# epfl-lts2/pygsp

Measured on AMD Instinct MI355X. Metric: filtered-vertices/sec (N·Nsig·K/s) + achieved HBM GB/s vs roofline, 1M-vertex K=30, higher is better.
Workload: dtype f64

## Files before the change

pygsp_amd/csrc/gspx_ctx.hip.h:

```cpp
#pragma once

struct Options {
  int64_t kernel = 0;
  int64_t vec = 0;
  int64_t rows_per_wave = 0;
  int64_t narrow_g_log2 = -1;
  int64_t waves_per_block = 4;
  int64_t calib_mix = 0;
  int64_t graph_launch = 2;
  int64_t tile_gather = 1;
  int64_t tile_workgroups = 0;
  int64_t knn_f32 = 1;
  int64_t tile_pad = 1;
  int64_t tile_min_row = 16;
  int64_t staged_copy = 1;
  int64_t staged_copy_min_mb = 32;
  int64_t copy_threads = 0;
  int64_t tile_regroup = 1;
  int64_t tile_acc_builds = 1;
  int64_t tile_lg = 0;
  int64_t edge_vertex_walk = 1;
  int64_t fuse_input = 1;
  int64_t tile_nt = -1;
  int64_t synthesis = 0;
  int64_t alternate_sweep = 1;
  int64_t xcd_remap = 1;
  int64_t combine = 0;
  int64_t ws_limit_mb = 65536;
  int64_t max_batch = 0;
  int64_t gather_rccl = 1;
  int64_t lds_pad_kb = 0;
  int64_t host_pipeline = 1;
  int64_t host_batch = 0;
  int64_t host_edge = 0;
  int64_t host_threads = 0;
  int64_t streamed_alloc = 1;
  int64_t layout_splits = 0;
};

struct gspx_ctx {
  int device = 0;
  int cu_count = 256;
  hipStream_t stream = nullptr;
  Options opt;
  DevMem ws_t;
  DevMem ws_r;
  DevMem ws_w;
  DevMem io_x, io_y;
  DevMem ws_spec;
  DevMem ws_sq, ws_sqp;
  HostPipe* pipe = nullptr;
  CopyStage* copy = nullptr;
  bool counted = false;
  std::mutex comms_mu;
  std::vector<struct gspx_comm*> comms;
  hipEvent_t ev[4] = {nullptr, nullptr, nullptr, nullptr};
  std::vector<hipEvent_t> ev_pool;
  double timing[5] = {0, 0, 0, 0, 0};
  int64_t step_kinds[2] = {0, 0};
  bool capturing = false;
  std::vector<unsigned char> seen_key;
  std::vector<unsigned char> graph_key;
  hipGraphExec_t graph_exec = nullptr;
  int64_t graph_kinds[2] = {0, 0};
};

static std::atomic<int> g_live_ctx[64];

static void replay_reset(gspx_ctx* ctx) {
  if (!ctx) return;
  ctx->seen_key.clear();
  ctx->graph_key.clear();
// ... 153 lines not shown
  ctx->ws_r.release();
  ctx->ws_w.release();
  ctx->io_x.release();
  ctx->io_y.release();
  ctx->ws_spec.release();
  ctx->ws_sq.release();
  ctx->ws_sqp.release();
  if (ctx->pipe) {
    ctx->pipe->destroy();
    delete ctx->pipe;
    ctx->pipe = nullptr;
  }
  if (ctx->copy) {
    ctx->copy->destroy();
    delete ctx->copy;
    ctx->copy = nullptr;
  }
  if (ctx->stream) (void)hipStreamDestroy(ctx->stream);
  delete ctx;
  return GSPX_OK;
}

extern "C" int gspx_ctx_sync(gspx_ctx* ctx) {
  if (!ctx) return set_err(GSPX_ERR_INVALID, "null ctx");
  HIPCHK(hipSetDevice(ctx->device));
  HIPCHK(hipStreamSynchronize(ctx->stream));
  return GSPX_OK;
}

struct OptionDef {
  const char* key;
  int64_t Options::*slot;
  bool (*ok)(int64_t);
  const char* refusal;
};
static const OptionDef OPTION_TABLE[] = {
    {"kernel", &Options::kernel, [](int64_t v) { return v == 0 || v == 1 || v == 2 || v == 5; },
     "kernel must be 0 (auto), 1 (panel), 2 (narrow) or 5 (LDS-staged)"},
    {"vec", &Options::vec, [](int64_t v) { return v == 0 || v == 1 || v == 2 || v == 4; }, "vec must be 0, 1, 2 or 4"},
    {"rows_per_wave", &Options::rows_per_wave, [](int64_t v) { return v >= 0 && v <= 1024; },
     "rows_per_wave must be in [0, 1024] (0 = auto)"},
    {"narrow_g_log2", &Options::narrow_g_log2, [](int64_t v) { return v >= -1 && v <= 6; },
     "narrow_g_log2 must be in [-1, 6] (-1 = auto)"},
    {"waves_per_block", &Options::waves_per_block, [](int64_t v) { return v == 4 || v == 8 || v == 16; },
     "waves_per_block must be 4, 8 or 16"},
    {"alternate_sweep", &Options::alternate_sweep, nullptr, nullptr},
    {"synthesis", &Options::synthesis, nullptr, nullptr},
    {"tile_gather", &Options::tile_gather, nullptr, nullptr},
    {"graph_launch", &Options::graph_launch, nullptr, nullptr},
    {"tile_workgroups", &Options::tile_workgroups, nullptr, nullptr},
    {"tile_lg", &Options::tile_lg, nullptr, nullptr},
    {"tile_regroup", &Options::tile_regroup, nullptr, nullptr},
    {"tile_acc_builds", &Options::tile_acc_builds, nullptr, nullptr},
    {"staged_copy", &Options::staged_copy, nullptr, nullptr},
    {"staged_copy_min_mb", &Options::staged_copy_min_mb, nullptr, nullptr},
    {"copy_threads", &Options::copy_threads, nullptr, nullptr},
    {"tile_min_row", &Options::tile_min_row, nullptr, nullptr},
    {"tile_pad", &Options::tile_pad, nullptr, nullptr},
    {"knn_f32", &Options::knn_f32, nullptr, nullptr},
    {"tile_nt", &Options::tile_nt, nullptr, nullptr},
    {"fuse_input", &Options::fuse_input, nullptr, nullptr},
    {"edge_vertex_walk", &Options::edge_vertex_walk, nullptr, nullptr},
    {"xcd_remap", &Options::xcd_remap, nullptr, nullptr},
    {"combine", &Options::combine, nullptr, nullptr},
    {"ws_limit_mb", &Options::ws_limit_mb, nullptr, nullptr},
    {"max_batch", &Options::max_batch, nullptr, nullptr},
    {"gather_rccl", &Options::gather_rccl, nullptr, nullptr},
    {"lds_pad_kb", &Options::lds_pad_kb, nullptr, nullptr},
    {"host_pipeline", &Options::host_pipeline, nullptr, nullptr},
    {"host_batch", &Options::host_batch, nullptr, nullptr},
    {"host_edge", &Options::host_edge, nullptr, nullptr},
    {"host_threads", &Options::host_threads, nullptr, nullptr},
    {"streamed_alloc", &Options::streamed_alloc, nullptr, nullptr},
    {"layout_splits", &Options::layout_splits, [](int64_t v) { return v >= 0 && v <= 65535; },
     "layout_splits must be in [0, 65535] (0 = automatic)"},
};

static const OptionDef* find_option(const char* key) {
  if (key)
    for (const OptionDef& d : OPTION_TABLE)
      if (!strcmp(key, d.key)) return &d;
  set_err(GSPX_ERR_INVALID, "unknown option '%s'", key ? key : "(null)");
  return nullptr;
}

extern "C" int gspx_ctx_set_option(gspx_ctx* ctx, const char* key, int64_t value) {
  replay_reset(ctx);
  if (!ctx) return set_err(GSPX_ERR_INVALID, "null ctx");
  const OptionDef* d = find_option(key);
  if (!d) return GSPX_ERR_INVALID;
  if (d->ok && !d->ok(value)) return set_err(GSPX_ERR_INVALID, "%s", d->refusal);
  ctx->opt.*d->slot = value;
  if (d->slot == &Options::streamed_alloc) {
    const bool on = value != 0;
    (void)hipSetDevice(ctx->device);
    for (DevMem* m : {&ctx->ws_t, &ctx->ws_r}) {
      if (!on && m->va_size) {
        (void)hipStreamSynchronize(ctx->stream);
        m->release();
      }
      m->streamed = on;
    }
  }
  return GSPX_OK;
}

// ... 200 lines not shown
```

pygsp_amd/csrc/gspx_poly.hip.h:

```cpp
#pragma once

struct PlanStep {
  double scale = 1.0, gamma = -1.0;
  int flush = 0;
  int final = 0;
  std::vector<double> w;
};

static void make_plan_fused(int nf, int M, const std::vector<double>& cp, bool acc_existing,
                            bool final_to_y, std::vector<PlanStep>& plan) {
  const int K = M - 1;
  plan.assign((size_t)K, PlanStep());
  int covered = -1;
  bool first = !acc_existing;
  for (int k = 1; k <= K; ++k) {
    PlanStep& st = plan[(size_t)k - 1];
    st.scale = (k == 1) ? 0.5 : 1.0;
    st.gamma = (k == 1) ? 0.0 : -1.0;
    st.w.assign((size_t)nf * 3, 0.0);
    const bool must = (k == K) || (k >= 2 && (k - 2) > covered);
    if (!must) continue;
    st.flush = first ? 1 : 2;
    first = false;
    st.final = (k == K && final_to_y) ? 1 : 0;
// ... 343 lines not shown
  return (int)std::max<int64_t>(1, std::min(std::min(tiles, want), fit));
}
static size_t cross_parts(const gspx_ctx* ctx, int N, unsigned w, int M, int nf) {
  size_t most = 0;
  for (int here : {std::min(nf, CROSS_PASS), nf % CROSS_PASS})
    for (int vec = 1; here > 0 && vec <= (w % 2 == 0 ? 2 : 1); ++vec)
      most = std::max(most, (size_t)cross_gx(ctx, N, w, M, here, vec) * (size_t)here * M * w);
  return most;
}

template <typename T>
static int launch_slot_cross_dots(gspx_ctx* ctx, const T* slots, int M, size_t slot_stride, unsigned pitch, int N,
                                  unsigned w, const int* perm, const CrossDots& cd, hipStream_t st) {
  const T* z = (const T*)cd.z;
  const int vec = cross_vec<T>(w, pitch, z, cd.ldz);
  const int cwl = sqnorm_cwl(w / vec);
  typedef void (*kern_t)(const T*, int, size_t, u32, const T*, int, size_t, u32, const int*, int, int, int, double*);
  for (int f0 = 0; f0 < cd.nf; f0 += CROSS_PASS) {
    const int here = std::min(CROSS_PASS, cd.nf - f0);
    const bool few = here <= CROSS_FEW;
    kern_t kern = few ? k_slot_cross_dots<T, 1, 16, CROSS_FEW> : k_slot_cross_dots<T, 1, 8, CROSS_PASS>;
    if constexpr (sizeof(T) == 4) {
      if (vec == 2) kern = few ? k_slot_cross_dots<T, 2, 8, CROSS_FEW> : k_slot_cross_dots<T, 2, 4, CROSS_PASS>;
    }
    const int gx = cross_gx(ctx, N, w, M, here, vec);
    const dim3 grid((unsigned)gx, (unsigned)cross_chunks(M, here, vec), (w / vec + (1u << cwl) - 1) >> cwl);
    hipLaunchKernelGGL(kern, grid, dim3(256), 0, st, slots, M, slot_stride, (u32)pitch, z + (size_t)f0 * cd.zplane, here,
                       cd.zplane, (u32)cd.ldz, perm, N, (int)w, cwl, cd.part);
    const int64_t n = (int64_t)here * M * w;
    hipLaunchKernelGGL(k_dots_reduce, dim3((unsigned)((n + 63) / 64)), dim3(256), 0, st, cd.part, gx, n, (int)w,
                       cd.out + (size_t)f0 * M * cd.ldo, cd.ldo);
  }
  return GSPX_OK;
}

struct SlotsUse {
  int (*fn)(gspx_ctx*, const void*, int, size_t, unsigned, int, unsigned, const int*, const void*, hipStream_t);
  const void* arg;
};

template <typename T> static bool tile_geometry(const gspx_graph* g, const Options& opt, unsigned ld) {
  constexpr int TVEC = 16 / (int)sizeof(T);
  const size_t U = (size_t)g->N * ld;
  return opt.tile_gather && g->gt_rows == GSPX_TILE_BR && (size_t)ld * sizeof(T) >= (size_t)opt.tile_min_row &&
         (ld % TVEC) == 0 && U * sizeof(T) < ((size_t)1 << 31) && (size_t)g->nnz_int * sizeof(T) < ((size_t)1 << 31);
}
template <typename T>
static bool tile_usable(const gspx_graph* g, const Options& opt, unsigned ld, const T* y, unsigned ldy) {
  constexpr int TVEC = 16 / (int)sizeof(T);
  return tile_geometry<T>(g, opt, ld) && (ldy % TVEC) == 0 && (((uintptr_t)y / sizeof(T)) % TVEC) == 0;
}
template <typename T>
static int launch_step_tile(gspx_graph* g, const Options& opt, TileArgs<T> t, unsigned ld, hipStream_t st,
                            const T* vals = nullptr) {
  const size_t rowb = (size_t)ld * sizeof(T);
  int lg = rowb <= 16 ? 1 : rowb <= 32 ? 2 : rowb <= 64 ? 4 : rowb <= 128 ? 8 : 16;
  if (opt.tile_lg == 8 || opt.tile_lg == 4 || opt.tile_lg == 2) lg = rowb <= 128 ? std::max(lg, (int)opt.tile_lg) : 16;
  const bool narrow = lg < 16;
  const int ncol = narrow ? 1 : (int)((rowb + 255) / 256);
  const int flavour = t.old_rows ? 1 : t.nin > 0 ? 2 : 0;
  typedef void (*kern_t)(const TileArgs<T>);
  static const kern_t wide[3][3] = {
      {k_step_tile<T, 0>, k_step_tile<T, 1>, k_step_tile<T, 2>},
      {k_step_tile<T, 0, 16, true>, k_step_tile<T, 1, 16, true>, k_step_tile<T, 2, 16, true>},
      {k_step_tile<T, 0, 16, false, true>, k_step_tile<T, 1, 16, false, true>, k_step_tile<T, 2, 16, false, true>}};
  static const kern_t slim[3][4] = {
      {k_step_tile<T, 1, 1, false, false, 64>, k_step_tile<T, 1, 2, false, false, 128>,
       k_step_tile<T, 1, 4, false, false, 256>, k_step_tile<T, 1, 8>},
      {k_step_tile<T, 1, 1, true, false, 64>, k_step_tile<T, 1, 2, true, false, 128>,
       k_step_tile<T, 1, 4, true, false, 256>, k_step_tile<T, 1, 8, true>},
      {k_step_tile<T, 1, 1, false, true, 64>, k_step_tile<T, 1, 2, false, true, 128>,
       k_step_tile<T, 1, 4, false, true, 256>, k_step_tile<T, 1, 8, false, true>}};
  kern_t kern = narrow ? slim[flavour][lg == 1 ? 0 : lg == 2 ? 1 : lg == 4 ? 2 : 3] : wide[flavour][ncol <= 2 ? ncol : 0];
  unsigned threads = narrow ? 64u * (unsigned)lg : 512u;
  const bool noacc = opt.tile_acc_builds && t.flush == 0 && !narrow && flavour == 0;
  if (noacc) {
    static const kern_t freek[3] = {k_step_tile<T, 0, 16, false, false, 512, 16, 0, false>,
                                    k_step_tile<T, 1, 16, false, false, 512, 16, 0, false>,
                                    k_step_tile<T, 2, 16, false, false, 512, 16, 0, false>};
    kern = freek[ncol <= 2 ? ncol : 0];
  }
  bool mix = false;
  if (opt.calib_mix && !narrow && flavour == 0) {
    static const kern_t mixk[2][3] = {
        {k_step_tile<T, 0, 16, false, false, 512, 16, 1>, k_step_tile<T, 1, 16, false, false, 512, 16, 1>,
         k_step_tile<T, 2, 16, false, false, 512, 16, 1>},
        {k_step_tile<T, 0, 16, false, false, 512, 16, 2>, k_step_tile<T, 1, 16, false, false, 512, 16, 2>,
         k_step_tile<T, 2, 16, false, false, 512, 16, 2>}};
    static const kern_t mixfree[2][3] = {
        {k_step_tile<T, 0, 16, false, false, 512, 16, 1, false>, k_step_tile<T, 1, 16, false, false, 512, 16, 1, false>,
         k_step_tile<T, 2, 16, false, false, 512, 16, 1, false>},
        {k_step_tile<T, 0, 16, false, false, 512, 16, 2, false>, k_step_tile<T, 1, 16, false, false, 512, 16, 2, false>,
         k_step_tile<T, 2, 16, false, false, 512, 16, 2, false>}};
    kern = (noacc ? mixfree : mixk)[opt.calib_mix == 2 ? 1 : 0][ncol <= 2 ? ncol : 0];
    mix = true;
  }
  const int pieces = (int)(rowb / 16);
  if (opt.tile_regroup && ncol == 1 && flavour != 1 && pieces < lg && !mix) {
#define GSPX_CL(LG_, CL_, NT_) \
  (flavour == 2 ? (kern_t)k_step_tile<T, 1, LG_, false, true, NT_, CL_> : (kern_t)k_step_tile<T, 1, LG_, false, false, NT_, CL_>)
    kern_t k2 = nullptr;
    unsigned nt2 = 0;
    if (lg == 4 && pieces == 3) k2 = GSPX_CL(4, 3, 192), nt2 = 192;
    else if (lg == 8 && pieces == 5) k2 = GSPX_CL(8, 5, 320), nt2 = 320;
    else if (lg == 16 && pieces == 10) k2 = GSPX_CL(16, 10, 320), nt2 = 320;
#undef GSPX_CL
    if (k2) kern = k2, threads = nt2;
  }
  size_t lds = g->gt_lds;
  if (lg < 8)
    lds = std::min(lds, (size_t)GSPX_TILE_MAXN1 * 16 * lg + (((size_t)g->gt_entmax * sizeof(T) + 15) & ~(size_t)15) +
                            (((size_t)g->gt_entmax + 15) & ~(size_t)15) + 64);
  if (lg < 8) lds = (lds + 2047) & ~(size_t)2047;
  int per_cu = 2;
  {
    struct Known { size_t attr = 0; std::map<size_t, int> fit; };
    static std::map<std::pair<const void*, int>, Known> known;
    static std::mutex lds_mu;
    std::lock_guard<std::mutex> lock(lds_mu);
    Known& k = known[std::make_pair((const void*)kern, g->ctx->device)];
    if (k.attr < lds) {
      HIPCHK(hipFuncSetAttribute((const void*)kern, hipFuncAttributeMaxDynamicSharedMemorySize, (int)lds));
      k.attr = lds;
    }
    if (lg < 8) {
      auto it = k.fit.find(lds);
      if (it == k.fit.end()) {
        int fit = 2;
        HIPCHK(hipOccupancyMaxActiveBlocksPerMultiprocessor(&fit, (const void*)kern, (int)threads, lds));
        it = k.fit.emplace(lds, std::max(2, std::min(fit, 16))).first;
      }
      per_cu = it->second;
    }
  }
// ... 93 lines not shown
  *width = max_ld;
  return GSPX_OK;
}

template <typename Batch>
static int run_batches(gspx_graph* g, int64_t Nsig, int64_t width, int steps, const Batch& batch) {
  gspx_ctx* ctx = g->ctx;
  size_t ev_idx = 0;
  HIPCHK(hipEventRecord(ctx->ev[0], ctx->stream));
  for (int64_t c0 = 0; c0 < Nsig; c0 += width)
    CHK(batch(c0, (unsigned)std::min<int64_t>(width, Nsig - c0), ev_idx));
  HIPCHK(hipEventRecord(ctx->ev[1], ctx->stream));
  HIPCHK(hipStreamSynchronize(ctx->stream));
  float ms = 0;
  HIPCHK(hipEventElapsedTime(&ms, ctx->ev[0], ctx->ev[1]));
  ctx->timing[0] = ms;
  double phase[3] = {0, 0, 0};
  for (size_t i = 0; i + 3 < ev_idx; i += 4)
    for (size_t j = 0; j < 3; ++j) {
      float t = 0;
      HIPCHK(hipEventElapsedTime(&t, ctx->ev_pool[i + j], ctx->ev_pool[i + j + 1]));
      phase[j] += t;
    }
  ctx->timing[1] = phase[1];
  ctx->timing[2] = (double)(ev_idx / 4) * steps;
  ctx->timing[3] = phase[0];
  ctx->timing[4] = phase[2];
  return GSPX_OK;
}

template <typename T>
static int run_batch(gspx_graph* g, int nf, int M, const std::vector<double>& cp, const T* x,
                     unsigned ldx, T* y, unsigned ldy, unsigned ld, bool deferred,
                     bool acc_existing, bool final_to_y, size_t& ev_idx, const SqNorms* sq = nullptr,
                     const SlotDots* sd = nullptr, const CrossDots* cd = nullptr, const SlotsUse* use = nullptr) {
  gspx_ctx* ctx = g->ctx;
  const Options& opt = ctx->opt;
  hipStream_t st = ctx->stream;
  const int N = (int)g->N;
  const int K = M - 1;
  const WorkPanels wp = work_panels<T>(g, opt, deferred || nf == 1, 1, ld, y, ldy);
  const bool tile_direct = wp.tile_direct, padded = wp.padded;
  const unsigned ldw = wp.ldw;
  const size_t U = (size_t)N * ldw;
  const Shape shape = choose_shape(opt, sizeof(T), ld, vec_cap(4, ldy, y));
  const int* perm = g->has_perm ? g->perm.as<int>() : nullptr;

  std::vector<PlanStep> plan;
  if (deferred)
    make_plan_deferred(nf, M, plan);
  else
    make_plan_fused(nf, M, cp, acc_existing, final_to_y, plan);

  std::vector<T> hw;
  if (deferred) {
    hw.resize((size_t)nf * M);
    for (size_t i = 0; i < hw.size(); ++i) hw[i] = (T)cp[i];
  } else {
    hw.resize((size_t)K * nf * 3);
    for (int k = 0; k < K; ++k)
      for (int j = 0; j < nf * 3; ++j) hw[(size_t)k * nf * 3 + j] = (T)plan[(size_t)k].w[(size_t)j];
  }
  const bool cap = ctx->capturing;
  if (!cap) {
    CHK(ctx->ws_w.ensure(hw.size() * sizeof(T) + 64));
    HIPCHK(hipMemcpyAsync(ctx->ws_w.p, hw.data(), hw.size() * sizeof(T), hipMemcpyHostToDevice, st));
    HIPCHK(hipStreamSynchronize(st));
  }

  const size_t nslots = deferred ? (size_t)M : 2;
  const size_t SU = U;
  CHK(ctx->ws_t.ensure(nslots * SU * sizeof(T) + 256));
  if (!deferred) CHK(ctx->ws_r.ensure((size_t)nf * U * sizeof(T) + 256));
  T* slots = ctx->ws_t.as<T>();
  T* racc = ctx->ws_r.as<T>();

  hipEvent_t ev[4] = {};
  if (!cap) CHK(batch_events(ctx, ev_idx, ev));
  const bool tile_ok = tile_direct || padded;
  const unsigned char* xb = (const unsigned char*)x;
  const unsigned char* yb = (const unsigned char*)y;
  const size_t xbytes = (size_t)N * ldx * sizeof(T), ybytes = (size_t)nf * N * ldy * sizeof(T);
  const bool fuse_in = tile_direct && !deferred && opt.fuse_input && g->gt_slow == 0 && ldx == ld &&
                       ((uintptr_t)x % 16) == 0 && (xb + xbytes <= yb || yb + ybytes <= xb) &&
                       (!g->has_perm || (g->gt_ns1 > 0 && (!cap || g->gt_s1nat.p)));
  if (fuse_in) {
    CHK(ensure_s1nat(g, st));
  } else if (padded) {
    const unsigned nb = (unsigned)std::min<size_t>((U + 255) / 256, 65536);
    hipLaunchKernelGGL((k_permute_in_pad<T>), dim3(nb), dim3(256), 0, st, x, ldx, slots, ldw, ld, N, perm);
  } else {
    launch_permute_in<T>(x, ldx, slots, ld, N, perm, vec_cap(shape.vec, ldx, x), st);
  }
  if (!cap) HIPCHK(hipEventRecord(ev[1], st));

  CHK(prepare_coff<T>(g, shape, ld, st));
  StepArgs<T> a = step_base<T>(g, ld, y, ldy);
  a.nf = nf;
  a.racc = racc;
  for (int k = 1; k <= K; ++k) {
    const PlanStep& ps = plan[(size_t)k - 1];
    if (tile_ok) {
      TileArgs<T> t{};
      if (deferred) {
        t.cur = slots + (size_t)(k - 1) * SU;
        t.old = (k >= 2 && ps.gamma != 0.0) ? slots + (size_t)(k - 2) * SU : t.cur;
        t.out = slots + (size_t)k * SU;
      } else {
        t.cur = slots + (size_t)((k - 1) & 1) * SU;
        t.old = ps.gamma == 0.0 ? t.cur : slots + (size_t)(k & 1) * SU;
        t.out = slots + (size_t)(k & 1) * SU;
        if (fuse_in && k == 1) {
          t.cur = x;
          t.old = x;
          t.s1rows = g->has_perm ? g->gt_s1nat.as<int>() : nullptr;
        } else if (fuse_in && k == 2) {
          t.old = x;
          t.old_rows = perm;
        }
      }
      t.racc = racc;
      t.y = y;
      t.ldy = ldy;
      t.perm = perm;
      t.scale = (T)ps.scale;
      t.gamma = (T)ps.gamma;
      t.beta = T(0);
      t.flush = ps.flush;
      t.final = padded ? 0 : ps.final;
      t.reverse = (opt.alternate_sweep && (k & 1)) ? 1 : 0;
      if (ps.flush) {
        t.wn = (T)ps.w[0];
        t.wc = (T)ps.w[1];
        t.wo = (T)ps.w[2];
      }
      CHK(launch_step_tile<T>(g, opt, t, ldw, st));
      continue;
    }
    if (deferred) {
      a.cur = slots + (size_t)(k - 1) * SU;
      a.old = k >= 2 ? slots + (size_t)(k - 2) * SU : slots;
      a.out = slots + (size_t)k * SU;
    } else {
      a.cur = slots + (size_t)((k - 1) & 1) * SU;
      a.old = slots + (size_t)(k & 1) * SU;
      a.out = slots + (size_t)(k & 1) * SU;
    }
    if (ps.gamma == 0.0) a.old = a.cur;
    a.scale = (T)ps.scale;
    a.gamma = (T)ps.gamma;
    a.flush = ps.flush;
    a.final = ps.final;
    a.reverse = (opt.alternate_sweep && (k & 1)) ? 1 : 0;
    a.wts = ctx->ws_w.as<T>() + (size_t)(k - 1) * nf * 3;
    launch_step<T>(ctx, a, shape, opt, st, g->coff.as<unsigned>());
  }
  if (!cap) HIPCHK(hipEventRecord(ev[2], st));
  if (deferred && sq) {
    CHK(launch_combine_sqnorm<T>(ctx, slots, M, SU, ldw, N, ld, *sq, st));
  } else if (deferred && sd) {
    CHK(launch_slot_dots<T>(ctx, slots, M, SU, ldw, N, ld, *sd, st));
  } else if (deferred && cd) {
    CHK(launch_slot_cross_dots<T>(ctx, slots, M, SU, ldw, N, ld, perm, *cd, st));
  } else if (deferred && use) {
    CHK(use->fn(ctx, slots, M, SU, ldw, N, ld, perm, use->arg, st));
  } else if (deferred) {
    launch_combine<T>(slots, M, SU, ctx->ws_w.as<T>(), M, nf, N, ld, y, ldy, (size_t)N * ldy, perm,
                      padded ? 1 : vec_cap(shape.vec, ldy, y), st, ldw);
  } else if (padded && final_to_y) {
    const unsigned nb = (unsigned)std::min<size_t>(((size_t)N * ld + 255) / 256, 65536);
    hipLaunchKernelGGL((k_permute_out_pad<T>), dim3(nb), dim3(256), 0, st, racc, ldw, y, ldy, ld, N, perm);
  }
  if (!cap) {
    HIPCHK(hipEventRecord(ev[3], st));
    HIPCHK(hipGetLastError());
  }
  return GSPX_OK;
}

template <typename T>
static int clenshaw_step(gspx_graph* g, const Options& opt, const WorkPanels& wp, const Shape& shape, StepArgs<T>& a,
                         int k, int K, const T* inp, const T* wts, int nin, const T* first, T* const B[2], T* y,
                         unsigned ldy, hipStream_t st) {
  gspx_ctx* ctx = g->ctx;
  const bool has_b2 = (k + 2 <= K);
  if (wp.tile_direct || wp.padded) {
    TileArgs<T> t{};
    t.cur = (k == K) ? first : B[(k + 1) & 1];
    t.old = (k < K && has_b2) ? B[k & 1] : t.cur;
// ... 52 lines not shown
  const size_t U = (size_t)N * ldw;
  const Shape shape = choose_shape(opt, sizeof(T), ld, vec_cap(4, ldy, y));
  const int* perm = g->has_perm ? g->perm.as<int>() : nullptr;

  std::vector<T> hw((size_t)M * nf);
  for (int k = 0; k < M; ++k)
    for (int f = 0; f < nf; ++f) hw[(size_t)k * nf + f] = (T)cp[(size_t)f * M + k];
  CHK(ctx->ws_w.ensure(hw.size() * sizeof(T) + 64));
  HIPCHK(hipMemcpyAsync(ctx->ws_w.p, hw.data(), hw.size() * sizeof(T), hipMemcpyHostToDevice, st));
  HIPCHK(hipStreamSynchronize(st));
  CHK(ctx->ws_r.ensure((size_t)nf * U * sizeof(T) + 256));
  CHK(ctx->ws_t.ensure(2 * U * sizeof(T) + 256));
  T* S = ctx->ws_r.as<T>();
  T* B[2] = {ctx->ws_t.as<T>(), ctx->ws_t.as<T>() + U};

  hipEvent_t ev[4];
  CHK(batch_events(ctx, ev_idx, ev));
  for (int f = 0; f < nf; ++f) {
    const T* xf = x + (size_t)f * plane_x;
    if (padded) {
      const unsigned nbp = (unsigned)std::min<size_t>((U + 255) / 256, 65536);
      hipLaunchKernelGGL((k_permute_in_pad<T>), dim3(nbp), dim3(256), 0, st, xf, ldx, S + (size_t)f * U, ldw, ld, N, perm);
      continue;
    }
    launch_permute_in<T>(xf, ldx, S + (size_t)f * U, ld, N, perm, vec_cap(shape.vec, ldx, xf), st);
  }
  HIPCHK(hipEventRecord(ev[1], st));

  CHK(prepare_coff<T>(g, shape, ld, st));
  StepArgs<T> a = step_base<T>(g, ld, y, ldy);
  for (int k = K; k >= 0; --k)
    CHK(clenshaw_step<T>(g, opt, wp, shape, a, k, K, S, ctx->ws_w.as<T>() + (size_t)k * nf, nf, S, B, y, ldy, st));
  HIPCHK(hipEventRecord(ev[2], st));
  if (padded) {
    const unsigned nbp = (unsigned)std::min<size_t>(((size_t)N * ld + 255) / 256, 65536);
    hipLaunchKernelGGL((k_permute_out_pad<T>), dim3(nbp), dim3(256), 0, st, B[0], ldw, y, ldy, ld, N, perm);
  }
  HIPCHK(hipEventRecord(ev[3], st));
  HIPCHK(hipGetLastError());
  return GSPX_OK;
}

template <typename T>
static int run_program_batch(gspx_graph* g, int S, const double* sc, const double* be, const double* ga, bool old_is_x,
                             const T* x, unsigned ldx, T* y, unsigned ldy, unsigned ld, size_t& ev_idx) {
  gspx_ctx* ctx = g->ctx;
  Options opt = ctx->opt;
  hipStream_t st = ctx->stream;
  const int N = (int)g->N;
  const size_t U = (size_t)N * ld;
  const Shape shape = choose_shape(opt, sizeof(T), ld, vec_cap(4, ldy, y));
  const int* perm = g->has_perm ? g->perm.as<int>() : nullptr;

  const T hw[3] = {T(1), T(0), T(0)};
  CHK(ctx->ws_w.ensure(sizeof(hw) + 64));
  HIPCHK(hipMemcpyAsync(ctx->ws_w.p, hw, sizeof(hw), hipMemcpyHostToDevice, st));
  HIPCHK(hipStreamSynchronize(st));
  CHK(ctx->ws_t.ensure((old_is_x ? 3 : 2) * U * sizeof(T) + 256));
  T* X = ctx->ws_t.as<T>();
  T* H[2] = {X + U, old_is_x ? X + 2 * U : X};

  hipEvent_t ev[4];
  CHK(batch_events(ctx, ev_idx, ev));
  launch_permute_in<T>(x, ldx, X, ld, N, perm, vec_cap(shape.vec, ldx, x), st);
  HIPCHK(hipEventRecord(ev[1], st));

  CHK(prepare_coff<T>(g, shape, ld, st));
  StepArgs<T> a = step_base<T>(g, ld, y, ldy);
  a.nf = 1;
  a.racc = H[0];
  a.wts = ctx->ws_w.as<T>();
  const bool tile_ok = tile_usable<T>(g, opt, ld, y, ldy);
  for (int s = 0; s < S; ++s) {
    const bool last = s == S - 1;
    const T* cur = (s == 0) ? X : H[(s - 1) & 1];
    T* out = H[s & 1];
    const T* old = old_is_x ? X : (const T*)out;
    const double gam = (!old_is_x && s == 0) ? 0.0 : ga[s];
    if (tile_ok) {
      TileArgs<T> t{};
      t.cur = cur;
      t.old = gam == 0.0 ? cur : old;
      t.out = out;
      t.racc = H[0];
      t.y = y;
      t.ldy = ldy;
      t.perm = perm;
      t.scale = (T)sc[s];
      t.beta = (T)be[s];
      t.gamma = (T)gam;
      t.flush = 0;
      t.final = last ? 1 : 0;
      t.reverse = (opt.alternate_sweep && (s & 1)) ? 1 : 0;
      CHK(launch_step_tile<T>(g, opt, t, ld, st));
      continue;
    }
    a.cur = cur;
    a.old = gam == 0.0 ? cur : old;
    a.out = out;
    a.scale = (T)sc[s];
    a.beta = (T)be[s];
    a.gamma = (T)gam;
    a.flush = last ? 1 : 0;
    a.final = last ? 1 : 0;
    a.reverse = (opt.alternate_sweep && (s & 1)) ? 1 : 0;
    launch_step<T>(ctx, a, shape, opt, st, g->coff.as<unsigned>());
  }
  HIPCHK(hipEventRecord(ev[2], st));
  HIPCHK(hipEventRecord(ev[3], st));
  HIPCHK(hipGetLastError());
  return GSPX_OK;
}

template <typename T>
static int filter_dev_t(gspx_graph* g, double lmax, int Nf, int M, const double* coeffs,
                        int64_t Nsig, const T* x, T* y, int mode) {
  gspx_ctx* ctx = g->ctx;
  const Options& opt = ctx->opt;
  const int64_t N = g->N;
  for (int i = 0; i < 5; ++i) ctx->timing[i] = 0;
  ctx->step_kinds[0] = ctx->step_kinds[1] = 0;
  if (N == 0 || Nsig == 0) return GSPX_OK;
  CHK(ensure_factor<T>(g, lmax));
  std::vector<double> cp;
  halve_c0(Nf, M, coeffs, cp);
// ... 463 lines not shown
```

pygsp_amd/csrc/gspx_tile_kernels.hip.h:

```cpp
#pragma once

#include "gspx_kernels.hip.h"

namespace gspx {

template <typename T> struct TileArgs {
  const int* rowptr;
  const int* col;
  const T* val;
  const int* hdr;
  const int* s1rows;
  const u8* lidx;
  const T* cur;
  const T* old;
  const int* old_rows;
  T* out;
  T* racc;
  T* y;
  const int* perm;
  int N;
  u32 ld, ldy;
  u32 panel_bytes, val_bytes, lidx_bytes;
  int nb, ncol, per_xcd;
  int lds_bytes;
  T scale, gamma;
  T beta;
  T wn, wc, wo;
  const T* inp;
  const T* wts;
  int nin;
  int flush;
  int final;
  int reverse;
  int nt;
};

constexpr int GSPX_TILE_BR = 64;
constexpr int GSPX_TILE_MAXN1 = 160;

template <typename T, int NCOL, int LG, bool OLDNAT, bool ACC = true> struct TileSchedule {
  static constexpr bool PF = !OLDNAT;
  static constexpr bool TILE_LAST = PF && LG == 16;
  static constexpr bool PF_ENTRIES = PF;
  static constexpr bool META_AFTER = !OLDNAT && LG == 16 && NCOL == 0;
  static constexpr bool EARLY_OLD = !ACC && PF && LG == 16 && NCOL == 2 && sizeof(T) == 4;
};

template <typename T, int NCOL, int LG = 16, bool OLDNAT = false, bool INS = false, int NT = 512, int CL = LG,
          int MIX = 0, bool ACC = true>
__global__ __launch_bounds__(NT, 4) void k_step_tile(const TileArgs<T> a) {
  static_assert(NT == 512 || (NT == 64 * LG && NCOL == 1) || (CL < LG && NCOL == 1 && NT % 64 == 0 && NT % CL == 0),
                "narrow builds: one row per group, one chunk per row");
  constexpr int BR = GSPX_TILE_BR;
  static_assert(CL <= LG && (BR % (NT / CL)) == 0, "compute groups must tile the block's rows");
  constexpr int MAXN1 = GSPX_TILE_MAXN1;
  typedef TileSchedule<T, NCOL, LG, OLDNAT, ACC> Sched;
  constexpr bool PF = Sched::PF;
  constexpr bool META_AFTER = Sched::META_AFTER;
  constexpr bool TILE_LAST = Sched::TILE_LAST;
  constexpr bool PF_ENTRIES = Sched::PF_ENTRIES;
  constexpr bool EARLY_OLD = Sched::EARLY_OLD;
  static_assert(ACC || (!OLDNAT && !INS && CL == LG), "flush-free builds: the plain flavour only");
  constexpr int VEC = 16 / (int)sizeof(T);
  typedef typename VT<T, VEC>::t V;
  typedef __attribute__((address_space(3))) void* lds_ptr;
  extern __shared__ __attribute__((aligned(16))) unsigned char gspx_smem[];

  const int tid = threadIdx.x;
  constexpr int NGD = NT / LG;
  constexpr int NG = NT / CL;
  constexpr int NE = (512 + NT - 1) / NT;
  constexpr int RPG = BR / NG;
  constexpr int ST = (MAXN1 + NGD - 1) / NGD;
  constexpr int RB = LG * 16;
  const int lane_d = tid & (LG - 1);
  const int grp_d = tid / LG;
  const int lane16 = CL == LG ? lane_d : tid % CL;
  const int grp = CL == LG ? grp_d : tid / CL;
  const int wave = tid >> 6;
  const int nwx = (int)(gridDim.x >> 3);
  const int xlo = (int)(blockIdx.x & 7) * a.per_xcd;
  int k1 = xlo + a.per_xcd;
  if (k1 > a.nb) k1 = a.nb;
  const int k0 = xlo + (int)(blockIdx.x >> 3);
  if (k0 >= k1) return;

  constexpr u32 POISON = 0x80000000u;
  const rsrc_t rcur = __builtin_amdgcn_make_buffer_rsrc((void*)a.cur, 0, a.panel_bytes, 0x00020000);
  const rsrc_t rold = __builtin_amdgcn_make_buffer_rsrc((void*)a.old, 0, a.panel_bytes, 0x00020000);
  const rsrc_t rra = __builtin_amdgcn_make_buffer_rsrc((void*)a.racc, 0, a.panel_bytes, 0x00020000);
  const rsrc_t rv = __builtin_amdgcn_make_buffer_rsrc((void*)a.val, 0, a.val_bytes, 0x00020000);
  const rsrc_t ri = __builtin_amdgcn_make_buffer_rsrc((void*)a.lidx, 0, a.lidx_bytes, 0x00020000);
  const u32 ldb = a.ld * (u32)sizeof(T);

  struct Meta { int rows[ST]; int rp[RPG + 1]; int orow[OLDNAT ? RPG : 1]; };
  const int xflip = xlo + k1 - 1;
  const bool rev = a.reverse != 0;
  auto phys = [&](int p) { return rev ? xflip - p : p; };
  auto load_hdr = [&](int p) { return *(const int4*)(a.hdr + (size_t)phys(p) * 4); };
  auto uniform = [](int4 h) {
    int4 u;
    u.x = __builtin_amdgcn_readfirstlane(h.x); u.y = __builtin_amdgcn_readfirstlane(h.y);
    u.z = __builtin_amdgcn_readfirstlane(h.z); u.w = __builtin_amdgcn_readfirstlane(h.w);
    return u;
  };
  auto load_meta = [&](int k, const int4& h) {
    Meta m;
    const int n1 = h.y;
#pragma unroll
    for (int t = 0; t < ST; ++t) {
      const int u = grp_d + NGD * t;
      m.rows[t] = a.s1rows[h.x + (u < n1 ? u : 0)];
    }
    int r = phys(k) * BR + grp * RPG;
#pragma unroll
// ... 84 lines not shown
  auto pass = [&](const int c, const bool first, const bool last, V (&ovc)[RPG], V (&ovn)[RPG])
                  __attribute__((always_inline)) {
    const int n1 = H.y, rp0 = H.z, ent = H.w;
    const bool fast = n1 >= 0;
    T* const mval = (T*)(tile + (fast ? n1 : 0) * LG);
    u8* const midx = (u8*)(mval + ent);
    const int row0 = phys(k) * BR + grp * RPG;
    int rs[RPG + 1];
#pragma unroll
    for (int t = 0; t < RPG + 1; ++t) rs[t] = M.rp[t] & ~3;
    const u32 col0 = (c * LG + lane16) * VEC;
    const bool on = col0 < a.ld;
    const u32 cb = on ? col0 * (u32)sizeof(T) : POISON;
    if constexpr (!PF) prefetch_rows(M, k, c, ovc);
    V ins[INS ? RPG : 1];
#pragma unroll
    for (int t = 0; t < (INS ? RPG : 1); ++t) ins[t] = 0;
    if constexpr (INS) {
      const rsrc_t rin = __builtin_amdgcn_make_buffer_rsrc((void*)a.inp, 0, a.panel_bytes * (u32)a.nin, 0x00020000);
      for (int f = 0; f < a.nin; ++f) {
        const T w = a.wts[f];
#pragma unroll
        for (int t = 0; t < RPG; ++t) {
          const u32 off = (row0 + t < a.N) ? (u32)(row0 + t) * ldb + cb : POISON;
          ins[t] += w * VT<T, VEC>::bload(rin, off == POISON ? POISON : off + (u32)f * a.panel_bytes);
        }
      }
    }
    if constexpr (!PF_ENTRIES) {
      if (first && fast) prefetch_entries(H);
    }
    int4 Hv = Hn;
    if constexpr (!META_AFTER) {
      if (last) {
        M = load_meta(kn < k1 ? kn : k, Hn);
        Hv = load_hdr(knn < k1 ? knn : k);
      }
    }
    __builtin_amdgcn_sched_barrier(0);
    if (first && fast) {
      const int nv16 = (ent * (int)sizeof(T) + 15) >> 4, ni16 = (ent + 15) >> 4;
#pragma unroll
      for (int q = 0; q < NE; ++q)
        if (tid + q * NT < nv16) *(u32x4*)((unsigned char*)mval + (tid + q * NT) * 16) = ev[q];
      if (tid < ni16) *(u32x4*)((unsigned char*)midx + tid * 16) = ei;
      for (int i = tid + NE * NT; i < nv16; i += NT)
        *(u32x4*)((unsigned char*)mval + i * 16) =
            __builtin_amdgcn_raw_buffer_load_b128(rv, (u32)rp0 * (u32)sizeof(T) + i * 16u, 0, 0);
      for (int i = tid + NT; i < ni16; i += NT)
        *(u32x4*)((unsigned char*)midx + i * 16) =
            __builtin_amdgcn_raw_buffer_load_b128(ri, (u32)rp0 + i * 16u, 0, 0);
    }
    if constexpr (TILE_LAST && !META_AFTER) {
      constexpr int NMETA = ST + RPG + 1 + 1;
      static_assert(NMETA < 16, "vmcnt immediate");
      if (last && !INS) __builtin_amdgcn_s_waitcnt(0x0070 | NMETA);
      else __builtin_amdgcn_s_waitcnt(0x0070);
    } else {
      __builtin_amdgcn_s_waitcnt(0x0070);
    }
    if constexpr (MIX != 2) __syncthreads();
    if constexpr (META_AFTER) {
      if (last) {
        M = load_meta(kn < k1 ? kn : k, Hn);
        Hv = load_hdr(knn < k1 ? knn : k);
      }
    }
    if constexpr (EARLY_OLD) {
      if ((!last || kn < k1) && a.gamma != T(0)) prefetch_rows(M, last ? kn : k, last ? 0 : c + 1, ovn);
    }
    __builtin_amdgcn_sched_barrier(0);
    V nv[RPG], res[ACC ? RPG : 1];
#pragma unroll
    for (int t = 0; t < RPG; ++t) {
      const int s = rs[t], e = rs[t + 1];
      V acc = 0, self = 0;
      if (MIX && fast) {
        self = tile[(int)midx[s - rp0] * LG + lane16];
        acc = mval[s - rp0] * self;
      } else if (fast) {
        acc = lds_row_dot<T, V, LG, u8>(mval + (s - rp0), midx + (s - rp0), row0 + t < a.N ? e - s : 0, tile, lane16,
                                        self);
      } else if (row0 + t < a.N) {
        for (int j = s; j < e; ++j) {
          const int cc = a.col[j];
          const V xv = VT<T, VEC>::bload(rcur, cc < a.N ? (u32)cc * ldb + cb : POISON);
          if (j == s) self = xv;
          acc += a.val[j] * xv;
        }
      }
      if constexpr (ACC) {
        nv[t] = a.scale * acc + a.gamma * ovc[t] + a.beta * self;
      } else {
        nv[t] = __builtin_elementwise_fma((V)a.beta, self, __builtin_elementwise_fma((V)a.gamma, ovc[t], a.scale * acc));
      }
      if constexpr (INS) nv[t] += ins[t];
      if constexpr (ACC) {
        res[t] = a.wn * nv[t] + a.wc * self + a.wo * ovc[t];
        if (a.flush == 2) res[t] += ra[t];
      }
    }
    __builtin_amdgcn_s_waitcnt(0xC07F);
    if constexpr (MIX != 2) __builtin_amdgcn_s_barrier();
    bool more = true;
    if (last) {
      const int4 Hnn = uniform(Hv);
      H = Hn;
      Hn = Hnn;
      more = kn < k1;
    }
    __builtin_amdgcn_sched_barrier(0);
    if constexpr (!PF) {
      if (more && H.y >= 0) stage(M, H.y, chunk_off_d(last ? 0 : c + 1));
    }
#pragma unroll
    for (int t = 0; t < RPG; ++t) {
      const int row = row0 + t;
      if (row < a.N && on) {
        if (a.final && (!ACC || !a.flush)) {
          const size_t orow = a.perm ? (size_t)a.perm[row] : (size_t)row;
          *(V*)(a.y + orow * a.ldy + col0) = nv[t];
          continue;
        }
        if (a.nt & 8) __builtin_nontemporal_store(nv[t], (V*)(a.out + (size_t)row * a.ld + col0));
        else *(V*)(a.out + (size_t)row * a.ld + col0) = nv[t];
        if constexpr (ACC) {
          if (a.flush) {
            if (a.final) {
              const size_t orow = a.perm ? (size_t)a.perm[row] : (size_t)row;
              *(V*)(a.y + orow * a.ldy + col0) = res[t];
            } else {
              if (a.nt & 2) __builtin_nontemporal_store(res[t], (V*)(a.racc + (size_t)row * a.ld + col0));
              else *(V*)(a.racc + (size_t)row * a.ld + col0) = res[t];
            }
          }
        }
      }
    }
    __builtin_amdgcn_sched_barrier(0);
    if constexpr (PF) {
      if (more) {
        const int nc = last ? 0 : c + 1;
        if constexpr (!TILE_LAST) {
          if (H.y >= 0) stage(M, H.y, chunk_off_d(nc));
        }
        if constexpr (!EARLY_OLD) prefetch_rows(M, last ? kn : k, nc, ovn);
        if constexpr (PF_ENTRIES) {
          if (last && H.y >= 0) prefetch_entries(H);
        }
        if constexpr (TILE_LAST) {
          __builtin_amdgcn_sched_barrier(0);
          if (H.y >= 0) stage(M, H.y, chunk_off_d(nc));
          __builtin_amdgcn_sched_barrier(0);
        }
      }
    }
    if (last) {
      k = kn;
      kn = knn;
      knn += nwx;
    }
    return more;
  };
  if constexpr (EARLY_OLD) {
    static_assert(NCOL == 2, "an even number of passes per block");
    for (;;) {
      pass(0, true, false, ov, ov2);
      if (!pass(1, false, true, ov2, ov)) break;
    }
  } else {
    for (;;) {
      if constexpr (NCOL == 1) {
        if (!pass(0, true, true, ov, ov)) break;
      } else if constexpr (NCOL == 2) {
        pass(0, true, false, ov, ov);
        if (!pass(1, false, true, ov, ov)) break;
      } else {
        bool more = true;
// ... 124 lines not shown
```

Before: 194.4 billion.

## Skip final T_k store, add prefetching OLDNAT tile builds, drop unused weight uploads

Adds a tile kernel variant (KEEP=false) for the last Chebyshev step that skips writing the T_k output rows when the step flushes to the accumulator, since nothing reads them. This removes one full-matrix HBM write per filter call. Adds AHEAD builds that turn on prefetching for the OLDNAT flavour and widen the vmcnt wait count to cover the extra old-row loads. It also skips the host-to-device weight copy and stream synchronize when the tile path takes its weights from kernel arguments, cutting host stalls. All of this is gated by a new tile_edge_builds option that defaults to on, and the bigger vmcnt immediate adds some risk.

After: 196.5 billion, median of 6. 1.1% higher.

```diff
diff --git a/pygsp_amd/csrc/gspx_ctx.hip.h b/pygsp_amd/csrc/gspx_ctx.hip.h
--- a/pygsp_amd/csrc/gspx_ctx.hip.h
+++ b/pygsp_amd/csrc/gspx_ctx.hip.h
@@ -18,6 +18,7 @@
   int64_t copy_threads = 0;
   int64_t tile_regroup = 1;
   int64_t tile_acc_builds = 1;
+  int64_t tile_edge_builds = 1;
   int64_t tile_lg = 0;
   int64_t edge_vertex_walk = 1;
   int64_t fuse_input = 1;
@@ -277,6 +278,7 @@
     {"tile_lg", &Options::tile_lg, nullptr, nullptr},
     {"tile_regroup", &Options::tile_regroup, nullptr, nullptr},
     {"tile_acc_builds", &Options::tile_acc_builds, nullptr, nullptr},
+    {"tile_edge_builds", &Options::tile_edge_builds, nullptr, nullptr},
     {"staged_copy", &Options::staged_copy, nullptr, nullptr},
     {"staged_copy_min_mb", &Options::staged_copy_min_mb, nullptr, nullptr},
     {"copy_threads", &Options::copy_threads, nullptr, nullptr},
diff --git a/pygsp_amd/csrc/gspx_poly.hip.h b/pygsp_amd/csrc/gspx_poly.hip.h
--- a/pygsp_amd/csrc/gspx_poly.hip.h
+++ b/pygsp_amd/csrc/gspx_poly.hip.h
@@ -419,7 +419,7 @@
 }
 template <typename T>
 static int launch_step_tile(gspx_graph* g, const Options& opt, TileArgs<T> t, unsigned ld, hipStream_t st,
-                            const T* vals = nullptr) {
+                            const T* vals = nullptr, bool last_step = false) {
   const size_t rowb = (size_t)ld * sizeof(T);
   int lg = rowb <= 16 ? 1 : rowb <= 32 ? 2 : rowb <= 64 ? 4 : rowb <= 128 ? 8 : 16;
   if (opt.tile_lg == 8 || opt.tile_lg == 4 || opt.tile_lg == 2) lg = rowb <= 128 ? std::max(lg, (int)opt.tile_lg) : 16;
@@ -447,6 +447,19 @@
                                     k_step_tile<T, 2, 16, false, false, 512, 16, 0, false>};
     kern = freek[ncol <= 2 ? ncol : 0];
   }
+  const bool nokeep = (opt.tile_edge_builds == 1 || opt.tile_edge_builds == 2) && last_step && t.flush != 0 && !narrow &&
+                      flavour == 0;
+  if (nokeep) {
+    static const kern_t lastk[3] = {k_step_tile<T, 0, 16, false, false, 512, 16, 0, true, false>,
+                                    k_step_tile<T, 1, 16, false, false, 512, 16, 0, true, false>,
+                                    k_step_tile<T, 2, 16, false, false, 512, 16, 0, true, false>};
+    kern = lastk[ncol <= 2 ? ncol : 0];
+  }
+  if ((opt.tile_edge_builds == 1 || opt.tile_edge_builds == 3) && !narrow && flavour == 1 && ncol <= 2) {
+    static const kern_t aheadk[2] = {k_step_tile<T, 1, 16, true, false, 512, 16, 0, true, true, true>,
+                                     k_step_tile<T, 2, 16, true, false, 512, 16, 0, true, true, true>};
+    kern = aheadk[ncol - 1];
+  }
   bool mix = false;
   if (opt.calib_mix && !narrow && flavour == 0) {
     static const kern_t mixk[2][3] = {
@@ -646,17 +659,18 @@
   else
     make_plan_fused(nf, M, cp, acc_existing, final_to_y, plan);
 
-  std::vector<T> hw;
-  if (deferred) {
-    hw.resize((size_t)nf * M);
-    for (size_t i = 0; i < hw.size(); ++i) hw[i] = (T)cp[i];
-  } else {
-    hw.resize((size_t)K * nf * 3);
-    for (int k = 0; k < K; ++k)
-      for (int j = 0; j < nf * 3; ++j) hw[(size_t)k * nf * 3 + j] = (T)plan[(size_t)k].w[(size_t)j];
-  }
   const bool cap = ctx->capturing;
-  if (!cap) {
+  const bool tile_ok = tile_direct || padded;
+  if (!cap && (deferred || !tile_ok)) {
+    std::vector<T> hw;
+    if (deferred) {
+      hw.resize((size_t)nf * M);
+      for (size_t i = 0; i < hw.size(); ++i) hw[i] = (T)cp[i];
+    } else {
+      hw.resize((size_t)K * nf * 3);
+      for (int k = 0; k < K; ++k)
+        for (int j = 0; j < nf * 3; ++j) hw[(size_t)k * nf * 3 + j] = (T)plan[(size_t)k].w[(size_t)j];
+    }
     CHK(ctx->ws_w.ensure(hw.size() * sizeof(T) + 64));
     HIPCHK(hipMemcpyAsync(ctx->ws_w.p, hw.data(), hw.size() * sizeof(T), hipMemcpyHostToDevice, st));
     HIPCHK(hipStreamSynchronize(st));
@@ -671,7 +685,6 @@
 
   hipEvent_t ev[4] = {};
   if (!cap) CHK(batch_events(ctx, ev_idx, ev));
-  const bool tile_ok = tile_direct || padded;
   const unsigned char* xb = (const unsigned char*)x;
   const unsigned char* yb = (const unsigned char*)y;
   const size_t xbytes = (size_t)N * ldx * sizeof(T), ybytes = (size_t)nf * N * ldy * sizeof(T);
@@ -728,7 +741,7 @@
         t.wc = (T)ps.w[1];
         t.wo = (T)ps.w[2];
       }
-      CHK(launch_step_tile<T>(g, opt, t, ldw, st));
+      CHK(launch_step_tile<T>(g, opt, t, ldw, st, nullptr, k == K && K > 2 && !deferred));
       continue;
     }
     if (deferred) {
@@ -887,10 +900,13 @@
   const Shape shape = choose_shape(opt, sizeof(T), ld, vec_cap(4, ldy, y));
   const int* perm = g->has_perm ? g->perm.as<int>() : nullptr;
 
-  const T hw[3] = {T(1), T(0), T(0)};
-  CHK(ctx->ws_w.ensure(sizeof(hw) + 64));
-  HIPCHK(hipMemcpyAsync(ctx->ws_w.p, hw, sizeof(hw), hipMemcpyHostToDevice, st));
-  HIPCHK(hipStreamSynchronize(st));
+  const bool tile_ok = tile_usable<T>(g, opt, ld, y, ldy);
+  if (!tile_ok) {
+    const T hw[3] = {T(1), T(0), T(0)};
+    CHK(ctx->ws_w.ensure(sizeof(hw) + 64));
+    HIPCHK(hipMemcpyAsync(ctx->ws_w.p, hw, sizeof(hw), hipMemcpyHostToDevice, st));
+    HIPCHK(hipStreamSynchronize(st));
+  }
   CHK(ctx->ws_t.ensure((old_is_x ? 3 : 2) * U * sizeof(T) + 256));
   T* X = ctx->ws_t.as<T>();
   T* H[2] = {X + U, old_is_x ? X + 2 * U : X};
@@ -905,7 +921,6 @@
   a.nf = 1;
   a.racc = H[0];
   a.wts = ctx->ws_w.as<T>();
-  const bool tile_ok = tile_usable<T>(g, opt, ld, y, ldy);
   for (int s = 0; s < S; ++s) {
     const bool last = s == S - 1;
     const T* cur = (s == 0) ? X : H[(s - 1) & 1];
diff --git a/pygsp_amd/csrc/gspx_tile_kernels.hip.h b/pygsp_amd/csrc/gspx_tile_kernels.hip.h
--- a/pygsp_amd/csrc/gspx_tile_kernels.hip.h
+++ b/pygsp_amd/csrc/gspx_tile_kernels.hip.h
@@ -38,8 +38,8 @@
 constexpr int GSPX_TILE_BR = 64;
 constexpr int GSPX_TILE_MAXN1 = 160;
 
-template <typename T, int NCOL, int LG, bool OLDNAT, bool ACC = true> struct TileSchedule {
-  static constexpr bool PF = !OLDNAT;
+template <typename T, int NCOL, int LG, bool OLDNAT, bool ACC = true, bool AHEAD = false> struct TileSchedule {
+  static constexpr bool PF = !OLDNAT || AHEAD;
   static constexpr bool TILE_LAST = PF && LG == 16;
   static constexpr bool PF_ENTRIES = PF;
   static constexpr bool META_AFTER = !OLDNAT && LG == 16 && NCOL == 0;
@@ -47,20 +47,23 @@
 };
 
 template <typename T, int NCOL, int LG = 16, bool OLDNAT = false, bool INS = false, int NT = 512, int CL = LG,
-          int MIX = 0, bool ACC = true>
+          int MIX = 0, bool ACC = true, bool KEEP = true, bool AHEAD = false>
 __global__ __launch_bounds__(NT, 4) void k_step_tile(const TileArgs<T> a) {
   static_assert(NT == 512 || (NT == 64 * LG && NCOL == 1) || (CL < LG && NCOL == 1 && NT % 64 == 0 && NT % CL == 0),
                 "narrow builds: one row per group, one chunk per row");
   constexpr int BR = GSPX_TILE_BR;
   static_assert(CL <= LG && (BR % (NT / CL)) == 0, "compute groups must tile the block's rows");
   constexpr int MAXN1 = GSPX_TILE_MAXN1;
-  typedef TileSchedule<T, NCOL, LG, OLDNAT, ACC> Sched;
+  typedef TileSchedule<T, NCOL, LG, OLDNAT, ACC, AHEAD> Sched;
   constexpr bool PF = Sched::PF;
   constexpr bool META_AFTER = Sched::META_AFTER;
   constexpr bool TILE_LAST = Sched::TILE_LAST;
   constexpr bool PF_ENTRIES = Sched::PF_ENTRIES;
   constexpr bool EARLY_OLD = Sched::EARLY_OLD;
   static_assert(ACC || (!OLDNAT && !INS && CL == LG), "flush-free builds: the plain flavour only");
+  static_assert(KEEP || (ACC && !OLDNAT && !INS && LG == 16 && CL == LG && MIX == 0),
+                "builds without the T_k store: the wide plain flavour with a flush");
+  static_assert(!AHEAD || (OLDNAT && LG == 16 && CL == LG && MIX == 0), "the pass-ahead OLDNAT builds: wide rows");
   constexpr int VEC = 16 / (int)sizeof(T);
   typedef typename VT<T, VEC>::t V;
   typedef __attribute__((address_space(3))) void* lds_ptr;
@@ -251,7 +254,7 @@
             __builtin_amdgcn_raw_buffer_load_b128(ri, (u32)rp0 + i * 16u, 0, 0);
     }
     if constexpr (TILE_LAST && !META_AFTER) {
-      constexpr int NMETA = ST + RPG + 1 + 1;
+      constexpr int NMETA = ST + RPG + 1 + 1 + (OLDNAT ? RPG : 0);
       static_assert(NMETA < 16, "vmcnt immediate");
       if (last && !INS) __builtin_amdgcn_s_waitcnt(0x0070 | NMETA);
       else __builtin_amdgcn_s_waitcnt(0x0070);
@@ -321,8 +324,10 @@
           *(V*)(a.y + orow * a.ldy + col0) = nv[t];
           continue;
         }
-        if (a.nt & 8) __builtin_nontemporal_store(nv[t], (V*)(a.out + (size_t)row * a.ld + col0));
-        else *(V*)(a.out + (size_t)row * a.ld + col0) = nv[t];
+        if constexpr (KEEP) {
+          if (a.nt & 8) __builtin_nontemporal_store(nv[t], (V*)(a.out + (size_t)row * a.ld + col0));
+          else *(V*)(a.out + (size_t)row * a.ld + col0) = nv[t];
+        }
         if constexpr (ACC) {
           if (a.flush) {
             if (a.final) {
```
